# lrmantovani10/Stable-Diffusion.mojo

Hardware: AMD Instinct MI355X
Metric: UNet denoising steps/sec @ 512x512 latent, batch=8 (higher is better)
Workload: dtype f16; 1 GPU; Tiny-SD UNet 512x512 (latent 4x64x64), batch 8/GPU, 50-step DDPM schedule, 77-token context, no CFG, random-init weights (BASELINE configs[1]); global_batch=8, parallelism=dp1 (independent prompts, weights broadcast once)

## Files before the change

### include/tsd.h

```cpp
#ifndef TSD_H
#define TSD_H

#include <stddef.h>
#include <stdint.h>

#ifdef __cplusplus
extern "C" {
#endif

#define TSD_VERSION 100

typedef enum tsd_status {
  TSD_OK = 0,
  TSD_E_ARG = -1,
  TSD_E_SHAPE = -2,
  TSD_E_ALLOC = -3,
  TSD_E_HIP = -4,
  TSD_E_RCCL = -5,
  TSD_E_STATE = -6,
  TSD_E_NONFINITE = -7
} tsd_status;

typedef struct tsd_ctx tsd_ctx;
typedef struct tsd_model tsd_model;
// ... 166 lines not shown
};
#define TSD_GD_VERSION_1 1
enum tsd_gemm_operand { TSD_GO_A0 = 0, TSD_GO_A1, TSD_GO_A2, TSD_GO_W, TSD_GO_WT1, TSD_GO_R, TSD_GO_BIAS, TSD_GO_ROWVEC, TSD_GO_C,
                        TSD_GO_VT, TSD_GO_GN, TSD_GO_COUNT };
int tsd_debug_gemm_record(tsd_ctx* ctx, int on);
int tsd_debug_gemm_recorded(tsd_ctx* ctx, int i, int64_t* desc, int n);
int tsd_debug_gemm_run(tsd_ctx* ctx, const int64_t* desc, int n, int cfg, const void* const* host_in, void* const* host_out,
                       int64_t* ext, int64_t* info);
enum tsd_norm_desc_field {
  TSD_ND_VERSION = 0, TSD_ND_MODE, TSD_ND_B, TSD_ND_HW, TSD_ND_C, TSD_ND_C0, TSD_ND_LD0, TSD_ND_LD1, TSD_ND_LDY, TSD_ND_GROUPS,
  TSD_ND_EPS, TSD_ND_GAMMA, TSD_ND_SILU, TSD_ND_HAS_W, TSD_ND_HAS_B, TSD_ND_TORCH_RSTD,
  TSD_ND_STATS, TSD_ND_NSLAB, TSD_ND_G0, TSD_ND_G1, TSD_ND_COMB, TSD_ND_ROWS,
  TSD_ND_COUNT
};
#define TSD_ND_VERSION_1 1
enum tsd_norm_mode { TSD_NM_GROUPNORM = 0, TSD_NM_GN_STATS, TSD_NM_GN_FINALIZE, TSD_NM_LAYERNORM };
enum tsd_norm_operand { TSD_NO_X0 = 0, TSD_NO_X1, TSD_NO_PART0, TSD_NO_PART1, TSD_NO_W, TSD_NO_BIAS, TSD_NO_Y, TSD_NO_STATS, TSD_NO_COUNT };
enum tsd_norm_info { TSD_NI_CHANGED = 0, TSD_NI_NSLAB, TSD_NI_OWN_PASS, TSD_NI_PREREDUCE, TSD_NI_FINALIZE, TSD_NI_COMPOSITE,
                     TSD_NI_SLAB_PIXELS, TSD_NI_APPLY_PIXELS, TSD_NI_PL, TSD_NI_COUNT };
int tsd_debug_norm_run(tsd_ctx* ctx, const int64_t* desc, int n, const void* const* host_in, void* const* host_out, int64_t* ext,
                       int64_t* info);
int tsd_debug_gn_path_counts(tsd_ctx* ctx, int64_t* counts, int n, int reset);
int tsd_debug_model_fold(tsd_model* m, int block, void* wf, float* bf);
int tsd_debug_attn_bench(tsd_ctx* ctx, int B, int H, int d, int Sq, int Sk, int iters, float* ms);
int tsd_debug_attn_exact_passes(tsd_ctx* ctx, int reset);
int tsd_debug_set_attn_qb(tsd_ctx* ctx, int mode);
int tsd_debug_set_attn_diag(tsd_ctx* ctx, int on);
int tsd_debug_set_res_fuse_skip(tsd_ctx* ctx, int on);
int tsd_debug_set_qkv_fuse(tsd_ctx* ctx, int on);
int tsd_debug_set_session_hoist(tsd_ctx* ctx, int on);
int tsd_debug_session_hoist_info(tsd_session* s, int64_t* info);
int tsd_debug_mfma_sustained(tsd_ctx* ctx, float ms_target, float* tflops, float* clock_ghz);

double tsd_flop_count(int kind, int L, int T);

#ifdef __cplusplus
}
#endif
#endif
```

### stable-diffusion.mojo_amd/csrc/common.h

```cpp
#pragma once
#include <hip/hip_runtime.h>
#include <stdint.h>
#include <stdio.h>
#include <string>
#include <vector>

#include "../../include/tsd.h"
#include "counter_rng.h"

typedef _Float16 half_t;

void tsd_set_error(const char* fmt, ...);
#define TSD_FAIL(code, ...)      \
  do {                           \
    tsd_set_error(__VA_ARGS__);  \
    return (code);               \
  } while (0)
#define HIP_TRY(expr)                                                                              \
  do {                                                                                             \
    hipError_t e__ = (expr);                                                                       \
    if (e__ != hipSuccess) TSD_FAIL(TSD_E_HIP, "%s failed: %s (%s:%d)", #expr, hipGetErrorString(e__), __FILE__, __LINE__); \
  } while (0)
#define TSD_TRY(expr)            \
  do {                           \
// ... 4 lines not shown
struct Arena {
  char* base = nullptr;
  size_t cap = 0, top = 0, peak = 0;
  bool planning = false;
  size_t mark() const { return top; }
  void release(size_t m) { top = m; }
  void* alloc(size_t bytes) {
    size_t a = (top + 255) & ~size_t(255);
    size_t n = a + bytes;
    if (n > peak) peak = n;
    if (!planning && n > cap) return nullptr;
    top = n;
    return planning ? (void*)(uintptr_t)(0x1000 + a) : (void*)(base + a);
  }
};

struct TsdOptions {
  int qkv_fuse = 1;
  int res_fuse_skip = 1;
  int gn_composite = 1;
  int conv_in_im2col = 1;
  int chain = 1;
  int fold_out = 1;
  int session_hoist = 1;
  int conv_w_tm_mib = 2, lin_w_tm = 1, lin_w_tm_kib = 1024;
  int attn_qb = 2;
  int attn_qb_force = 0;
  int attn_wg8 = 1;
  int attn8_var = 0;
  int attn_diag = 1;
  int attn_xcd = 0;
  int xcdn = 0, conv_halo = 0, splitk = 1, splitk_mink = 4096, splitk_tiles = 256, splitk_small = 8, splitk_wide = 1, splitk_ring4 = 0,
      splitk_big = 0, sk_cfg = 5, thin_cfg = 0, tune = 15, sk256 = 0, skip128 = 1;
  int force_cfg = -1;
  int sk_big_graph = 0;
  char cfg_override[512] = "";
  int gn_apply_mult = 2;
  int gn_finalize_min = 2048;
  int debug_occ = 0;
  int debug_poison_what = 7;
  int debug_poison = -1;
  int bench_wrot = 1, bench_epi = 0, bench_altcfg = -1, gemm_ts = 0;
  unsigned gen = 0;
};
void options_from_env(TsdOptions& o);

// ... 287 lines not shown
```

### stable-diffusion.mojo_amd/csrc/graph.cpp

```cpp
#include <math.h>

#include "graph.h"

#define CHECK_ALLOC(p) \
  if (!(p)) TSD_FAIL(TSD_E_ALLOC, "workspace arena exhausted (%s:%d)", __FILE__, __LINE__)

static int zero_async(tsd_ctx* ctx, void* p, size_t bytes) {
  if (!ctx->launch()) return TSD_OK;
  HIP_TRY(hipMemsetAsync(p, 0, bytes, ctx->stream));
  return TSD_OK;
}

Act act_alloc_gn(tsd_ctx* ctx, int B, int H, int W, int C, int groups) {
  Act a = act_alloc(ctx, B, H, W, C);
  if (a.p && groups > 0 && C % groups == 0) {
    a.gn_buf = arena_alloc<float>(ctx, (int64_t)B * ceil_div(H * W, 32) * groups * 2);
    a.gn_groups = a.gn_buf ? groups : 0;
  }
  return a;
}

static void gn_emit(const tsd_ctx* ctx, GemmArgs& g, Act* dst, int rows_per_sample) {
  if (!dst || !dst->gn_buf || dst->gn_groups <= 0 || g.N != dst->C || (g.epi & (EPI_OUT_F32 | EPI_GEGLU))) return;
  const int ns = gemm_gnstats_slabs(ctx, g.M, g.N, g.K, g.batch, g.conv, rows_per_sample, dst->gn_groups);
// ... 67 lines not shown
}

static NormSrc norm_src(const CatSrc& x, int C) {
  NormSrc s;
  s.x0 = x.p0; s.ld0 = x.ld0; s.C0 = x.C0;
  if (x.p1 && C > x.C0) { s.x1 = x.p1; s.ld1 = x.ld1; }
  return s;
}

extern "C" int tsd_debug_set_res_fuse_skip(tsd_ctx* ctx, int on) {
  return ctx_set_option(ctx, &TsdOptions::res_fuse_skip, on, 0, 1);
}

int g_resblock(tsd_ctx* ctx, const CatSrc& x, int B, int Hin, int Win, int ups, const ResW& w, const float* tvec,
               int tld, Act& out) {
  const int cin = w.cin, cout = w.cout;
  if (cin % 64 || cout % 64) TSD_FAIL(TSD_E_SHAPE, "residual block: channels (%d,%d) must be multiples of 64", cin, cout);
  if (cin > x.C0 + (x.p1 ? x.C1 : 0)) TSD_FAIL(TSD_E_SHAPE, "residual block: input has fewer than %d channels", cin);
  if (x.p1 && cin > x.C0 && (x.C0 % 64)) TSD_FAIL(TSD_E_SHAPE, "residual block: concat split %d not a multiple of 64", x.C0);
  if (!w.has_skip && (ups || (x.p1 && cin > x.C0))) TSD_FAIL(TSD_E_SHAPE, "residual block: identity skip needs a plain input");
  const int H = ups ? 2 * Hin : Hin, W = ups ? 2 * Win : Win;
  const size_t mark = ctx->arena.mark();
  Act h = act_alloc(ctx, B, Hin, Win, cin); CHECK_ALLOC(h.p);
  const bool x_stats = !(x.p1 && cin > x.C0) && x.gn_part0 && x.gn_groups0 == w.groups && x.C0 == cin;
  GnComposite gc;
  if (ctx->opt.gn_composite && x.p1 && cin == x.C0 + x.C1 && x.gn_part0 && x.gn_part1 && x.gn_groups0 > 0 && x.gn_groups1 > 0 &&
      x.gn_nslab0 == x.gn_nslab1 && x.gn_nslab0 > 0 && x.C0 % x.gn_groups0 == 0 && x.C1 % x.gn_groups1 == 0 && cin % w.groups == 0) {
    const int cf = x.C0 / x.gn_groups0, cpg = cin / w.groups;
    if (cf == x.C1 / x.gn_groups1 && cpg % cf == 0) {
      gc.part0 = x.gn_part0; gc.G0 = x.gn_groups0; gc.part1 = x.gn_part1; gc.G1 = x.gn_groups1; gc.nslab = x.gn_nslab0; gc.comb = cpg / cf;
    }
  }
  TSD_TRY(launch_groupnorm(ctx, norm_src(x, cin), B, Hin * Win, cin, w.groups, w.eps, 1.f, 1, h.p, h.ld,
                           x_stats ? x.gn_part0 : nullptr, x.gn_nslab0, w.gn1.w ? &w.gn1 : nullptr, gc.part0 ? &gc : nullptr));
  Act t1 = act_alloc_gn(ctx, B, H, W, cout, w.groups); CHECK_ALLOC(t1.p);
  TSD_TRY(g_conv3x3(ctx, h, w.conv1, 1, 1, 1, ups, tvec ? tvec + w.time_off : nullptr, tld, nullptr, 0, false, t1.p, t1.ld, &t1));
  Act h3 = act_alloc(ctx, B, H, W, cout); CHECK_ALLOC(h3.p);
  TSD_TRY(launch_groupnorm(ctx, norm_src(cat1(t1), cout), B, H * W, cout, w.groups, w.eps, 1.f, 1, h3.p, h3.ld, t1.gn_part,
                           t1.gn_nslab, w.gn2.w ? &w.gn2 : nullptr));
  Act r;
  if (w.has_skip && !ups && ctx->opt.res_fuse_skip > 0 && w.skip.k == 1 && w.skip.Ipad % 64 == 0 && w.skip.Ipad == cin &&
      !(x.p1 && cin > x.C0 && (x.C0 % 64))) {
    TSD_TRY(g_conv3x3(ctx, h3, w.conv2, 1, 1, 1, 0, nullptr, 0, nullptr, 0, false, out.p, out.ld, &out, &x, &w.skip));
    ctx->arena.release(mark);
    return TSD_OK;
  }
  if (w.has_skip) {
    r = act_alloc(ctx, B, Hin, Win, cout); CHECK_ALLOC(r.p);
    TSD_TRY(g_linear(ctx, x, (int64_t)B * Hin * Win, w.skip.w, w.skip.Ipad, cout, w.skip.Ipad, w.skip.b, nullptr, 0, 0,
                     r.p, r.ld));
  } else {
    r.p = const_cast<half_t*>(x.p0); r.ld = x.ld0; r.B = B; r.H = Hin; r.W = Win; r.C = cout;
  }
  TSD_TRY(g_conv3x3(ctx, h3, w.conv2, 1, 1, 1, 0, nullptr, 0, &r, ups, false, out.p, out.ld, &out));
  ctx->arena.release(mark);
  return TSD_OK;
// ... 313 lines not shown
  }
  auto attn = [&](int i) -> int {
    TSD_TRY(alloc_out(i, a[i - 1].H, a[i - 1].C));
    const AttnW& w = u.attn[i - 1];
    CtxKV kv;
    kv.K = kc_all + w.kv_off; kv.ldk = CK; kv.sK = (int64_t)Tp * CK;
    kv.Vt = vtc_all + (int64_t)w.kv_off * Tp; kv.ldvt = Tp; kv.sVt = (int64_t)CK * Tp;
    return g_unet_attn(ctx, a[i - 1], w, ctx16, T, Tp, a[i], &kv);
  };
  TSD_TRY(alloc_out(1, L, 320));
  if (in_im2col) TSD_TRY(g_linear(ctx, cat1(x0), (int64_t)B * L * L, u.conv_in_im2col, 64, u.conv1.Opad, 64, u.conv1.b, nullptr, 0, 0, a[1].p,
                                  a[1].ld, &a[1], L * L));
  else TSD_TRY(g_conv3x3(ctx, x0, u.conv1, 1, 1, 1, 0, nullptr, 0, nullptr, 0, false, a[1].p, a[1].ld, &a[1]));
  TSD_TRY(res(2, cat1(a[1]), L, 0));
  TSD_TRY(attn(3));
  TSD_TRY(alloc_out(4, L1, 320));
  TSD_TRY(g_conv3x3(ctx, a[3], u.conv4, 2, 1, 1, 0, nullptr, 0, nullptr, 0, false, a[4].p, a[4].ld, &a[4]));
  TSD_TRY(res(5, cat1(a[4]), L1, 0));
  TSD_TRY(attn(6));
  TSD_TRY(alloc_out(7, L2, 640));
  TSD_TRY(g_conv3x3(ctx, a[6], u.conv7, 2, 1, 1, 0, nullptr, 0, nullptr, 0, false, a[7].p, a[7].ld, &a[7]));
  TSD_TRY(res(8, cat1(a[7]), L2, 0));
  TSD_TRY(attn(9));
  TSD_TRY(res(10, cat2(a[9], a[9]), L2, 0));
  TSD_TRY(attn(11));
  TSD_TRY(res(12, cat2(a[11], a[7]), L2, 0));
  TSD_TRY(attn(13));
  TSD_TRY(res(15, cat1(a[13]), L2, 1));
  a[14] = a[15];
  TSD_TRY(attn(16));
  TSD_TRY(res(17, cat2(a[16], a[4]), L1, 0));
  TSD_TRY(attn(18));
  TSD_TRY(res(20, cat1(a[18]), L1, 1));
  a[19] = a[20];
  TSD_TRY(attn(21));
  TSD_TRY(res(22, cat2(a[21], a[1]), L, 0));
  TSD_TRY(attn(23));
  Act hf = act_alloc(ctx, B, L, L, 320); CHECK_ALLOC(hf.p);
  TSD_TRY(launch_groupnorm(ctx, norm_src(cat1(a[23]), 320), B, L * L, 320, 320, 1e-5f, 1.f, 1, hf.p, hf.ld,
                           a[23].gn_groups == 320 ? a[23].gn_part : nullptr, a[23].gn_nslab));
  if (eps_nhwc && u.final_conv.Opad == 4)
    return g_conv3x3(ctx, hf, u.final_conv, 1, 1, 1, 0, nullptr, 0, nullptr, 0, true, eps_out_chw, 4);
  float* eps_tmp = arena_alloc<float>(ctx, (int64_t)B * L * L * 4); CHECK_ALLOC(eps_tmp);
  TSD_TRY(g_conv3x3(ctx, hf, u.final_conv, 1, 1, 1, 0, nullptr, 0, nullptr, 0, true, eps_tmp, 4));
  TSD_TRY(launch_nhwc_f32_to_chw_f32(ctx, eps_tmp, B, 4, L, L, 4, eps_out_chw));
  return TSD_OK;
// ... 249 lines not shown
```

### stable-diffusion.mojo_amd/csrc/model.cpp

```cpp
#include <math.h>
#include <string.h>

#include "model.h"

bool attn_tail_weights_ok(const AttnW& w) {
  const int C = w.C;
  const bool plain = !w.ln[1].w && !w.ln[1].b && !w.ln[2].w && !w.ln[2].b && !w.gelu_erf;
  return plain && C == 320 && w.n_head == 8 && w.n_embed == 40 && w.sa_out.b && w.ca_out.b && w.geglu1.b && w.geglu2.b &&
         w.conv_out.b && !w.ca_q.b && w.sa_out.Kpad == C && w.ca_q.Kpad == C && w.ca_out.Kpad == C && w.geglu1.Kpad == C &&
         w.geglu2.Kpad == 4 * C && w.conv_out.Ipad == C && w.conv_out.k == 1;
}

bool attn_head_weights_ok(const AttnW& w) {
  const int C = w.C;
  return C == 320 && w.n_head == 8 && w.n_embed == 40 && !w.gn.w && !w.gn.b && !w.ln[0].w && !w.ln[0].b && w.conv_in.b &&
         w.conv_in.k == 1 && w.conv_in.Ipad == C && w.conv_in.Opad == C && !w.sa_in.b && w.sa_in.Kpad == C && w.sa_in.N == 3 * C;
}

static void model_invalidate_derived(tsd_model* m) {
  m->ready = false;
  m->gen++;
  for (auto& a : m->unet.attn) { a.tail_stream = nullptr; a.head_stream = nullptr; a.fold_w = nullptr; a.fold_w_tm = nullptr; a.fold_b = nullptr; }
  m->unet.conv_in_im2col = nullptr;
  m->vae.conv_in_im2col = nullptr;
  for (auto& r : m->unet.res) { r.conv1.w_tm = nullptr; r.conv2.w_tm = nullptr; }
  m->unet.conv4.w_tm = nullptr; m->unet.conv7.w_tm = nullptr; m->unet.kproj_all.w_tm = nullptr;
  for (auto& cv : m->unet.conv) cv.w_tm = nullptr;
  for (auto& a : m->unet.attn) {
    for (LinW* l : {&a.sa_in, &a.sa_out, &a.ca_q, &a.ca_out, &a.geglu1, &a.geglu2}) l->w_tm = nullptr;
    a.conv_in.w_tm = nullptr; a.conv_out.w_tm = nullptr;
  }
}

static size_t packed_bytes(const ParamSpec& p) {
  if (!p.used) return 0;
  switch (p.kind) {
    case P_CONV_W: return (size_t)p.Opad * p.shape[2] * p.shape[3] * p.Kpad * sizeof(half_t);
    case P_CONV_B: return (size_t)p.Opad * sizeof(float);
    case P_LIN_W: return (size_t)p.shape[0] * p.Kpad * sizeof(half_t);
    default: return (size_t)p.shape[0] * sizeof(float);
  }
}

extern "C" int tsd_model_create(tsd_ctx* ctx, int kind, tsd_model** out) {
// ... 126 lines not shown
      if (m->derived) HIP_TRY(hipFree(m->derived));
      m->derived = nullptr; m->derived_bytes = 0;
      hipError_t e = hipMalloc((void**)&m->derived, need);
      if (e != hipSuccess) TSD_FAIL(TSD_E_ALLOC, "derived weights: hipMalloc(%zu) failed: %s", need, hipGetErrorString(e));
      m->derived_bytes = need;
      if (ctx->opt.debug_poison >= 0 && (ctx->opt.debug_poison_what & 2)) HIP_TRY(hipMemsetAsync(m->derived, ctx->opt.debug_poison & 255, need, ctx->stream));
    }
    const bool wp = ctx->arena.planning;
    ctx->arena.planning = false;
    const int r = launch_pack_im2col_w(ctx, c0.w, c0.Opad, c0.Ipad, c0.I, (half_t*)m->derived);
    ctx->arena.planning = wp;
    if (r == TSD_OK) m->vae.conv_in_im2col = (const half_t*)m->derived;
    return r;
  }
  if (!is_diffusion_kind(m->kind)) return TSD_OK;
  std::vector<AttnW*> el;
  for (auto& a : m->unet.attn) if (a.C && (attn_tail_weights_ok(a) || attn_head_weights_ok(a))) el.push_back(&a);
  const ConvW& cin = is_full_unet_kind(m->kind) ? (m->unet.conv.empty() ? m->unet.conv1 : m->unet.conv[0]) : m->unet.conv1;
  const bool cin_ok = cin.w && cin.k == 3 && cin.I > 0 && 9 * cin.I <= 64 && cin.Ipad == 64;
  const size_t cin_b = cin_ok ? ((size_t)cin.Opad * 64 * sizeof(half_t) + 255) & ~size_t(255) : 0;
  const int tm_mib = ctx->opt.conv_w_tm_mib;
  const int tml_kib = ctx->opt.lin_w_tm_kib;
  const size_t tml_bytes = (size_t)(tml_kib > 0 ? tml_kib : 1024) << 10;
  std::vector<ConvW*> tm;
  size_t tm_b = 0;
  if (tm_mib > 0)
    for (auto& r : m->unet.res)
      for (ConvW* c : {&r.conv1, &r.conv2})
        if (c->w && c->k == 3 && (size_t)c->Opad * 9 * c->Ipad * 2 >= (size_t)tm_mib << 20) { tm.push_back(c); tm_b += (((size_t)c->Opad * 9 * c->Ipad * 2) + 255) & ~size_t(255); }
  if (tm_mib > 0) {
    for (ConvW* c : {&m->unet.conv4, &m->unet.conv7})
      if (c->w && c->k == 3 && (size_t)c->Opad * 9 * c->Ipad * 2 >= (size_t)tm_mib << 20) { tm.push_back(c); tm_b += (((size_t)c->Opad * 9 * c->Ipad * 2) + 255) & ~size_t(255); }
    for (auto& cv : m->unet.conv)
      if (cv.w && cv.k == 3 && (size_t)cv.Opad * 9 * cv.Ipad * 2 >= (size_t)tm_mib << 20) { tm.push_back(&cv); tm_b += (((size_t)cv.Opad * 9 * cv.Ipad * 2) + 255) & ~size_t(255); }
  }
  if (tm_mib > 0 && ctx->opt.lin_w_tm != 0)
    for (auto& a : m->unet.attn)
      if (a.C && !(attn_tail_weights_ok(a) && attn_head_weights_ok(a)))
        for (ConvW* c : {&a.conv_in, &a.conv_out})
          if (c->w && c->k == 1 && c->Ipad % 64 == 0 && (size_t)c->Opad * c->Ipad * 2 >= tml_bytes) { tm.push_back(c); tm_b += (((size_t)c->Opad * c->Ipad * 2) + 255) & ~size_t(255); }
  const int tml_mib = ctx->opt.lin_w_tm;
  std::vector<LinW*> tml;
  if (tml_mib > 0)
    for (auto& a : m->unet.attn)
      if (a.C && !(attn_tail_weights_ok(a) && attn_head_weights_ok(a)))
        for (LinW* l : {&a.sa_in, &a.sa_out, &a.ca_q, &a.ca_out, &a.geglu1, &a.geglu2})
          if (l->w && l->Kpad % 64 == 0 && l->Kpad == l->K && (size_t)l->N * l->Kpad * 2 >= tml_bytes) { tml.push_back(l); tm_b += (((size_t)l->N * l->Kpad * 2) + 255) & ~size_t(255); }
  LinW* kv = nullptr;
  if (tml_mib > 0 && m->unet.kproj_all.w && m->unet.vproj_all.w == m->unet.kproj_all.w + (int64_t)m->unet.kproj_all.N * m->unet.kproj_all.Kpad &&
      m->unet.kproj_all.Kpad % 64 == 0 && m->unet.vproj_all.N == m->unet.kproj_all.N) {
    kv = &m->unet.kproj_all;
    tm_b += (((size_t)2 * kv->N * kv->Kpad * 2) + 255) & ~size_t(255);
  }
  std::vector<AttnW*> fold;
  size_t fold_b = 0;
  if (ctx->opt.fold_out)
    for (auto& a : m->unet.attn)
      if (a.C && !attn_tail_weights_ok(a) && a.geglu2.w && a.conv_out.w && a.conv_out.k == 1 && a.conv_out.Ipad == a.C && a.conv_out.Opad == a.C &&
          a.geglu2.N == a.C && a.geglu2.Kpad == 4 * a.C && a.geglu2.K == 4 * a.C && a.C % 64 == 0) {
        fold.push_back(&a);
        fold_b += 2 * ((((size_t)a.C * 5 * a.C * 2) + 255) & ~size_t(255)) + ((((size_t)a.C * 4) + 255) & ~size_t(255));
      }
  if (el.empty() && !cin_ok && tm.empty() && tml.empty() && !kv && fold.empty()) return TSD_OK;
  const size_t tail_b = (attn_tail_stream_bytes() + 255) & ~size_t(255), head_b = (attn_head_stream_bytes() + 255) & ~size_t(255);
  const size_t each = tail_b + head_b, need = each * el.size() + cin_b + tm_b + fold_b;
  HIP_TRY(hipSetDevice(ctx->device));
  if (m->derived_bytes < need) {
    if (m->derived) HIP_TRY(hipFree(m->derived));
    m->derived = nullptr; m->derived_bytes = 0;
    hipError_t e = hipMalloc((void**)&m->derived, need);
    if (e != hipSuccess) TSD_FAIL(TSD_E_ALLOC, "derived weights: hipMalloc(%zu) failed: %s", need, hipGetErrorString(e));
    m->derived_bytes = need;
    if (ctx->opt.debug_poison >= 0 && (ctx->opt.debug_poison_what & 2)) HIP_TRY(hipMemsetAsync(m->derived, ctx->opt.debug_poison & 255, need, ctx->stream));
  }
  const bool was_planning = ctx->arena.planning;
  ctx->arena.planning = false;
  int r = TSD_OK;
  for (size_t i = 0; i < el.size() && r == TSD_OK; i++) {
    AttnW& a = *el[i];
    half_t* dst = (half_t*)(m->derived + i * each);
    if (attn_tail_weights_ok(a)) {
      r = launch_attn_tail_pack(ctx, a.sa_out.w, a.sa_out.Kpad, a.ca_q.w, a.ca_q.Kpad, a.ca_out.w, a.ca_out.Kpad, a.geglu1.w,
                                a.geglu1.Kpad, a.geglu2.w, a.geglu2.Kpad, a.conv_out.w, a.conv_out.Ipad, dst);
      if (r == TSD_OK) a.tail_stream = dst;
    }
    if (r == TSD_OK && attn_head_weights_ok(a)) {
      half_t* hd = (half_t*)(m->derived + i * each + tail_b);
      r = launch_attn_head_pack(ctx, a.conv_in.w, a.conv_in.Ipad, a.sa_in.w, a.sa_in.Kpad, hd);
// ... 18 lines not shown
      half_t* dst = (half_t*)(m->derived + off);
      r = launch_pack_tile_major(ctx, kv->w, 2 * kv->N, kv->Kpad, dst);
      if (r == TSD_OK) kv->w_tm = dst;
      off += (((size_t)2 * kv->N * kv->Kpad * 2) + 255) & ~size_t(255);
    }
    for (size_t i = 0; i < tml.size() && r == TSD_OK; i++) {
      LinW* l = tml[i];
      half_t* dst = (half_t*)(m->derived + off);
      r = launch_pack_tile_major(ctx, l->w, l->N, l->Kpad, dst);
      if (r == TSD_OK) l->w_tm = dst;
      off += (((size_t)l->N * l->Kpad * 2) + 255) & ~size_t(255);
    }
    for (size_t i = 0; i < fold.size() && r == TSD_OK; i++) {
      AttnW* a = fold[i];
      const int C = a->C;
      const size_t wb = (((size_t)C * 5 * C * 2) + 255) & ~size_t(255);
      half_t* wf = (half_t*)(m->derived + off);
      half_t* wf_tm = (half_t*)(m->derived + off + wb);
      float* bf = (float*)(m->derived + off + 2 * wb);
      r = launch_fold_linear_conv1x1(ctx, a->conv_out.w, a->conv_out.Ipad, a->conv_out.b, a->geglu2.w, a->geglu2.Kpad, a->geglu2.b, C, 4 * C, wf, 5 * C, bf);
      if (r == TSD_OK) r = launch_pack_tile_major(ctx, wf, C, 5 * C, wf_tm);
      if (r == TSD_OK) { a->fold_w = wf; a->fold_w_tm = wf_tm; a->fold_b = bf; }
      off += 2 * wb + ((((size_t)C * 4) + 255) & ~size_t(255));
    }
  }
  if (r == TSD_OK && !fold.empty()) {
    hipError_t e = hipStreamSynchronize(ctx->stream);
    for (size_t i = 0; i < fold.size() && r == TSD_OK && e == hipSuccess; i++) {
      const AttnW* a = fold[i];
      const int C = a->C;
      std::vector<uint16_t> hw((size_t)C * 5 * C);
      std::vector<float> hb(C);
      e = hipMemcpy(hw.data(), a->fold_w, hw.size() * 2, hipMemcpyDeviceToHost);
      if (e == hipSuccess) e = hipMemcpy(hb.data(), a->fold_b, hb.size() * 4, hipMemcpyDeviceToHost);
      if (e != hipSuccess) break;
      int64_t bad = 0;
      for (uint16_t v : hw) bad += (v & 0x7C00) == 0x7C00;
      for (float v : hb) bad += !(fabsf(v) <= 3.4028235e38f);
      if (bad) {
        fold[i]->fold_w = nullptr; fold[i]->fold_w_tm = nullptr; fold[i]->fold_b = nullptr;
        tsd_set_error("attention block with C = %d: %lld folded weights / biases are not finite (W_out . W_2 leaves fp16)", C, (long long)bad);
        r = TSD_E_NONFINITE;
      }
    }
    if (e != hipSuccess && r == TSD_OK) {
      tsd_set_error("fold check: %s", hipGetErrorString(e));
// ... 14 lines not shown
  return TSD_OK;
}

extern "C" int tsd_model_prepare(tsd_model* m) {
  if (!m) TSD_FAIL(TSD_E_ARG, "NULL model");
  HIP_TRY(hipSetDevice(m->ctx->device));
  TSD_TRY(model_check_ready(m));
  HIP_TRY(hipStreamSynchronize(m->ctx->stream));
  return TSD_OK;
}

extern "C" int tsd_debug_model_fold(tsd_model* m, int block, void* wf, float* bf) {
  if (!m) TSD_FAIL(TSD_E_ARG, "NULL model");
  if (!is_diffusion_kind(m->kind) || block < 0 || block >= (int)m->unet.attn.size())
    TSD_FAIL(TSD_E_ARG, "model_fold: no attention block %d in this model", block);
  HIP_TRY(hipSetDevice(m->ctx->device));
  TSD_TRY(model_check_ready(m));
  const AttnW& a = m->unet.attn[block];
  if (!a.fold_w) return 0;
  HIP_TRY(hipStreamSynchronize(m->ctx->stream));
  if (wf) HIP_TRY(hipMemcpy(wf, a.fold_w, (size_t)a.C * 5 * a.C * 2, hipMemcpyDeviceToHost));
  if (bf) HIP_TRY(hipMemcpy(bf, a.fold_b, (size_t)a.C * 4, hipMemcpyDeviceToHost));
  return a.C;
}

ConvW model_conv(const tsd_model* m, const std::string& prefix) {
  ConvW w;
  auto it = m->index.find(prefix + ".kernel");
  if (it == m->index.end()) return w;
  const ParamSpec& pw = m->params[it->second];
  const ParamSpec& pb = m->params[it->second + 1];
  if (!pw.used) return w;
  w.w = (const half_t*)(m->blob + pw.off);
  w.b = (const float*)(m->blob + pb.off);
  w.O = (int)pw.shape[0]; w.I = (int)pw.shape[1]; w.k = (int)pw.shape[2]; w.Ipad = pw.Kpad; w.Opad = pw.Opad;
  return w;
}

LinW model_lin(const tsd_model* m, const std::string& prefix, bool use_bias) {
  LinW w;
  auto it = m->index.find(prefix + ".weight");
  if (it == m->index.end()) return w;
  const ParamSpec& pw = m->params[it->second];
  const ParamSpec& pb = m->params[it->second + 1];
  w.w = (const half_t*)(m->blob + pw.off);
  w.b = (use_bias && pb.used) ? (const float*)(m->blob + pb.off) : nullptr;
// ... 141 lines not shown
```

### stable-diffusion.mojo_amd/csrc/model.h

```cpp
#pragma once
#include <map>
#include <string>
#include <vector>

#include "common.h"

enum ParamKind { P_CONV_W = 0, P_CONV_B = 1, P_LIN_W = 2, P_LIN_B = 3 };

struct ParamSpec {
  std::string name;
  int64_t shape[4] = {0, 0, 0, 0};
  int ndim = 0;
  int kind = 0;
  bool used = true;
  float bound = 0.f;
  float offset = 0.f;
  int Opad = 0, Kpad = 0;
  int interleave = 0;
  int region = 0;
  size_t off = 0, bytes = 0;
  int64_t numel() const {
    int64_t n = 1;
    for (int i = 0; i < ndim; i++) n *= shape[i];
    return n;
// ... 3 lines not shown
enum LayerKind { L_CONV, L_CONV_S2, L_RES, L_ATTN, L_UP, L_GN, L_SILU, L_UPCONV };
struct LayerDef { int kind; int a, b, c, d; };
extern const LayerDef UNET_LAYERS[23];
extern const LayerDef DECODER_LAYERS[26];
extern const LayerDef ENCODER_LAYERS[19];
enum { U_POP = 1, U_PUSH = 2 };
struct UNetStep { LayerDef l; int flags; };
constexpr int SD15_N = 45;
extern const UNetStep SD15_STEPS[SD15_N];
static inline bool is_full_unet_kind(int kind) { return kind == TSD_MODEL_DIFFUSION_SD15 || kind == TSD_MODEL_DIFFUSION_SD15_TORCH; }
static inline bool is_diffusion_kind(int kind) { return kind == TSD_MODEL_DIFFUSION || is_full_unet_kind(kind); }
static inline bool is_clip_kind(int kind) { return kind == TSD_MODEL_CLIP || kind == TSD_MODEL_CLIP_TORCH; }
static inline bool is_decoder_kind(int kind) { return kind == TSD_MODEL_DECODER || kind == TSD_MODEL_DECODER_TORCH; }
static inline bool is_encoder_kind(int kind) { return kind == TSD_MODEL_ENCODER || kind == TSD_MODEL_ENCODER_TORCH; }
static inline bool is_vae_torch_kind(int kind) { return kind == TSD_MODEL_DECODER_TORCH || kind == TSD_MODEL_ENCODER_TORCH; }
constexpr int TSD_MODEL_KIND_MAX = TSD_MODEL_ENCODER_TORCH;

std::vector<ParamSpec> build_param_specs(int model_kind);

struct ResW {
  ConvW conv1, conv2, skip;
  LinW time;
  int cin = 0, cout = 0, groups = 32;
  bool has_skip = false;
  int time_off = 0;
  NormAffine gn1, gn2;
  float eps = 1e-5f;
};
struct AttnW {
  int n_head = 0, n_embed = 0, C = 0, d_ctx = 768;
  ConvW conv_in, conv_out;
  LinW sa_in, sa_out, ca_q, ca_k, ca_v, ca_out, geglu1, geglu2;
  int kv_off = 0;
  NormAffine gn, ln[3];
  bool gelu_erf = false;
  const half_t* tail_stream = nullptr;
  const half_t* head_stream = nullptr;
  const half_t* fold_w = nullptr; const half_t* fold_w_tm = nullptr; const float* fold_b = nullptr;
};
bool attn_tail_weights_ok(const AttnW& w);
bool attn_head_weights_ok(const AttnW& w);
struct VaeAttnW {
  int C = 0;
  LinW in_proj, out_proj;
  NormAffine gn;
  float eps = 1e-5f;
};

struct UNetW {
  LinW t1, t2;
  LinW tproj;
  LinW kproj_all, vproj_all;
  ConvW conv1, conv4, conv7, final_conv;
  const half_t* conv_in_im2col = nullptr;
  std::vector<ResW> res;
  std::vector<AttnW> attn;
  std::vector<ConvW> conv;
  NormAffine final_gn;
  int final_groups = 320;
};
struct VaeW {
  std::vector<ConvW> conv;
  const half_t* conv_in_im2col = nullptr;
  std::vector<ResW> res;
  std::vector<VaeAttnW> attn;
  std::vector<NormAffine> gn;
  float gn_eps = 1e-5f;
};

struct ClipLayerW { LinW in_proj, out_proj, l4, l5; NormAffine ln1, ln2; };
struct ClipW {
  const half_t* tok = nullptr;
  const float* pos = nullptr;
  ClipLayerW layer[12];
  NormAffine final_ln;
};

struct PlanKey { int B, L, T; bool operator<(const PlanKey& o) const { return B != o.B ? B < o.B : (L != o.L ? L < o.L : T < o.T); } };

struct tsd_model {
// ... 22 lines not shown
```

### stable-diffusion.mojo_amd/csrc/runtime.cpp

```cpp
#include <stdarg.h>
#include <stdlib.h>
#include <string.h>

#include "common.h"

static thread_local char g_err[512] = "";

void tsd_set_error(const char* fmt, ...) {
  va_list ap;
  va_start(ap, fmt);
  vsnprintf(g_err, sizeof(g_err), fmt, ap);
  va_end(ap);
}

static int env_int(const char* name, int dflt) { const char* e = getenv(name); return e && *e ? atoi(e) : dflt; }
void options_from_env(TsdOptions& o) {
  o.qkv_fuse = env_int("TSD_QKV_FUSE", o.qkv_fuse);
  o.res_fuse_skip = env_int("TSD_RES_FUSE_SKIP", o.res_fuse_skip);
  o.gn_composite = env_int("TSD_GN_COMPOSITE", o.gn_composite);
  o.conv_in_im2col = env_int("TSD_CONV_IN_IM2COL", o.conv_in_im2col);
  o.chain = env_int("TSD_CHAIN", o.chain) ? 1 : 0;
  o.fold_out = env_int("TSD_FOLD_OUT", o.fold_out) ? 1 : 0;
  o.session_hoist = env_int("TSD_SESSION_HOIST", o.session_hoist) ? 1 : 0;
  o.conv_w_tm_mib = env_int("TSD_CONV_W_TM", o.conv_w_tm_mib);
  o.lin_w_tm = env_int("TSD_LIN_W_TM", o.lin_w_tm);
  o.lin_w_tm_kib = env_int("TSD_LIN_W_TM_KIB", o.lin_w_tm_kib);
  { const int q = env_int("TSD_ATTN_QB", o.attn_qb); if (q == 1 || q == 2) o.attn_qb = q; }
  o.attn_xcd = env_int("TSD_ATTN_XCD", o.attn_xcd);
  o.attn_wg8 = env_int("TSD_ATTN_WG8", o.attn_wg8) ? 1 : 0;
  o.attn8_var = env_int("TSD_ATTN8_VAR", o.attn8_var);
  o.xcdn = env_int("TSD_GEMM_XCDN", o.xcdn);
  o.conv_halo = env_int("TSD_CONV_HALO", o.conv_halo);
  o.splitk = env_int("TSD_GEMM_SPLITK", o.splitk);
  o.splitk_mink = env_int("TSD_GEMM_SPLITK_MINK", o.splitk_mink);
  o.splitk_tiles = env_int("TSD_GEMM_SPLITK_TILES", o.splitk_tiles);
  o.splitk_small = env_int("TSD_GEMM_SPLITK_SMALL", o.splitk_small);
  o.splitk_wide = env_int("TSD_GEMM_SPLITK_WIDE", o.splitk_wide);
  o.splitk_ring4 = env_int("TSD_GEMM_SPLITK_RING4", o.splitk_ring4);
  o.splitk_big = env_int("TSD_GEMM_SPLITK_BIG", o.splitk_big);
  o.sk_cfg = env_int("TSD_GEMM_SK_CFG", o.sk_cfg);
  o.sk256 = env_int("TSD_GEMM_SK256", o.sk256);
  o.thin_cfg = env_int("TSD_GEMM_THIN_CFG", o.thin_cfg);
  o.skip128 = env_int("TSD_GEMM_SKIP128", o.skip128);
  o.tune = env_int("TSD_GEMM_TUNE", o.tune);
  if (const char* ov = getenv("TSD_GEMM_CFG_OVERRIDE")) { strncpy(o.cfg_override, ov, sizeof(o.cfg_override) - 1); o.cfg_override[sizeof(o.cfg_override) - 1] = 0; }
// ... 185 lines not shown
```

### stable-diffusion.mojo_amd/tsd/_lib.py

```python
import ctypes as C
import os

import numpy as np

_HERE = os.path.dirname(os.path.abspath(__file__))
LIB_PATH = os.environ.get("TSD_LIB") or os.path.join(os.path.dirname(_HERE), "lib", "libtsd.so")

TSD_OK, TSD_E_ARG, TSD_E_SHAPE, TSD_E_ALLOC, TSD_E_HIP, TSD_E_RCCL, TSD_E_STATE, TSD_E_NONFINITE = 0, -1, -2, -3, -4, -5, -6, -7
os.environ.setdefault("HIP_FORCE_DEV_KERNARG", "1")

MODEL_DIFFUSION, MODEL_DECODER, MODEL_ENCODER, MODEL_CLIP, MODEL_DIFFUSION_SD15, MODEL_DIFFUSION_SD15_TORCH = 1, 2, 3, 4, 5, 6
MODEL_CLIP_TORCH, MODEL_DECODER_TORCH, MODEL_ENCODER_TORCH = 7, 8, 9
SAMPLER_KINDS = {"ddpm": 0, "ddim": 1, "dpmpp_2m": 2}
TIMESTEP_SPACINGS = {"leading": 0, "trailing": 1}
MASK_MODES = {"area": 0, "any": 1}


def sampler_kind(kind):
    return SAMPLER_KINDS.get(kind.lower(), -1) if isinstance(kind, str) else int(kind)


def timestep_spacing(spacing):
    return TIMESTEP_SPACINGS.get(spacing.lower(), -1) if isinstance(spacing, str) else int(spacing)

# ... 92 lines not shown
        "tsd_session_download_latents": ([vp, fp], i), "tsd_session_download_images": ([vp, i, fp], i),
        "tsd_dist_unique_id": ([vp], i), "tsd_dist_init": ([vp, i, i, vp], i),
        "tsd_dist_broadcast_weights": ([vp, i], i), "tsd_dist_finalize": ([vp], i),
        "tsd_dist_comm_count": ([vp, C.POINTER(i)], i),
        "tsd_flop_count": ([i, i, i], C.c_double),
        "tsd_debug_splitk_errors": ([vp], i),
        "tsd_debug_xcd_round_robin": ([], i),
        "tsd_debug_nonfinite_count": ([vp, i], i),
        "tsd_debug_set_fused_attention": ([vp, i], i),
        "tsd_debug_gemm_bench": ([vp, i, i, i, i, i, i, i, i, i, i, fp], i),
        "tsd_debug_attn_bench": ([vp, i, i, i, i, i, i, fp], i),
        "tsd_debug_attn_exact_passes": ([vp, i], i),
        "tsd_debug_set_attn_qb": ([vp, i], i),
        "tsd_debug_set_attn_diag": ([vp, i], i),
        "tsd_debug_set_res_fuse_skip": ([vp, i], i),
        "tsd_debug_set_qkv_fuse": ([vp, i], i),
        "tsd_debug_set_session_hoist": ([vp, i], i),
        "tsd_debug_session_hoist_info": ([vp, C.POINTER(i64)], i),
        "tsd_debug_mfma_sustained": ([vp, C.c_float, fp, fp], i),
        "tsd_debug_gemm_check": ([vp, i, i, i, i, i, i, i, i, i, i, fp, fp], i),
        "tsd_debug_gemm_record": ([vp, i], i),
        "tsd_debug_gemm_recorded": ([vp, i, C.POINTER(i64), i], i),
        "tsd_debug_model_fold": ([vp, i, vp, fp], i),
        "tsd_debug_gemm_run": ([vp, C.POINTER(i64), i, i, C.POINTER(vp), C.POINTER(vp), C.POINTER(i64), C.POINTER(i64)], i),
        "tsd_debug_norm_run": ([vp, C.POINTER(i64), i, C.POINTER(vp), C.POINTER(vp), C.POINTER(i64), C.POINTER(i64)], i),
        "tsd_debug_gn_path_counts": ([vp, C.POINTER(i64), i, i], i),
    }
    for name, (args, res) in sig.items():
        fn = getattr(l, name)
        fn.argtypes = args
        fn.restype = res


EXPORTS = None


def declared_symbols():
    import re
    hdr = os.path.join(os.path.dirname(os.path.dirname(_HERE)), "include", "tsd.h")
    txt = open(hdr).read()
    txt = re.sub(r"/\*.*?\*/", "", txt, flags=re.S)
    return sorted(set(re.findall(r"\b(tsd_[a-z0-9_]+)\s*\(", txt)))


def last_error():
    return lib().tsd_last_error().decode()
# ... 84 lines not shown
```

Before: 213.5 steps/s.

## Fold duplicated-concat residual block weights to halve input channels

In the Tiny-SD UNet, layer 10's residual block takes cat(a9, a9), the same activation concatenated with itself. The change sums the two input-channel halves of the conv1 and skip weights on the host at model prep time, and sets groups_in to half the groups. The block then runs on a9 alone with half the input channels, which removes half the GEMM K work and the concat read for that block. GroupNorm on the duplicated input is equivalent with half the groups, and it can reuse upstream stats through a new composite path. The costs are one-time host prep, extra derived weight memory, and fp16 rounding of the summed weights.

Result: faster. 217.0 steps/s, median of 6 (+1.6%).

```diff
diff --git a/include/tsd.h b/include/tsd.h
--- a/include/tsd.h
+++ b/include/tsd.h
@@ -212,6 +212,8 @@
                        int64_t* info);
 int tsd_debug_gn_path_counts(tsd_ctx* ctx, int64_t* counts, int n, int reset);
 int tsd_debug_model_fold(tsd_model* m, int block, void* wf, float* bf);
+int tsd_debug_model_dup_fold(tsd_model* m, void* conv1_w, void* skip_w);
+int64_t tsd_debug_dup_fold_host(const void* w, int rows, int taps, int ldw, int half, void* out, int ldo);
 int tsd_debug_attn_bench(tsd_ctx* ctx, int B, int H, int d, int Sq, int Sk, int iters, float* ms);
 int tsd_debug_attn_exact_passes(tsd_ctx* ctx, int reset);
 int tsd_debug_set_attn_qb(tsd_ctx* ctx, int mode);
diff --git a/stable-diffusion.mojo_amd/csrc/common.h b/stable-diffusion.mojo_amd/csrc/common.h
--- a/stable-diffusion.mojo_amd/csrc/common.h
+++ b/stable-diffusion.mojo_amd/csrc/common.h
@@ -50,6 +50,7 @@
   int conv_in_im2col = 1;
   int chain = 1;
   int fold_out = 1;
+  int fold_dup = 1;
   int session_hoist = 1;
   int conv_w_tm_mib = 2, lin_w_tm = 1, lin_w_tm_kib = 1024;
   int attn_qb = 2;
diff --git a/stable-diffusion.mojo_amd/csrc/graph.cpp b/stable-diffusion.mojo_amd/csrc/graph.cpp
--- a/stable-diffusion.mojo_amd/csrc/graph.cpp
+++ b/stable-diffusion.mojo_amd/csrc/graph.cpp
@@ -113,16 +113,20 @@
   const int H = ups ? 2 * Hin : Hin, W = ups ? 2 * Win : Win;
   const size_t mark = ctx->arena.mark();
   Act h = act_alloc(ctx, B, Hin, Win, cin); CHECK_ALLOC(h.p);
-  const bool x_stats = !(x.p1 && cin > x.C0) && x.gn_part0 && x.gn_groups0 == w.groups && x.C0 == cin;
+  const int g_in = w.groups_in > 0 ? w.groups_in : w.groups;
+  const bool x_stats = !(x.p1 && cin > x.C0) && x.gn_part0 && x.gn_groups0 == g_in && x.C0 == cin;
   GnComposite gc;
   if (ctx->opt.gn_composite && x.p1 && cin == x.C0 + x.C1 && x.gn_part0 && x.gn_part1 && x.gn_groups0 > 0 && x.gn_groups1 > 0 &&
-      x.gn_nslab0 == x.gn_nslab1 && x.gn_nslab0 > 0 && x.C0 % x.gn_groups0 == 0 && x.C1 % x.gn_groups1 == 0 && cin % w.groups == 0) {
-    const int cf = x.C0 / x.gn_groups0, cpg = cin / w.groups;
+      x.gn_nslab0 == x.gn_nslab1 && x.gn_nslab0 > 0 && x.C0 % x.gn_groups0 == 0 && x.C1 % x.gn_groups1 == 0 && cin % g_in == 0) {
+    const int cf = x.C0 / x.gn_groups0, cpg = cin / g_in;
     if (cf == x.C1 / x.gn_groups1 && cpg % cf == 0) {
       gc.part0 = x.gn_part0; gc.G0 = x.gn_groups0; gc.part1 = x.gn_part1; gc.G1 = x.gn_groups1; gc.nslab = x.gn_nslab0; gc.comb = cpg / cf;
     }
-  }
-  TSD_TRY(launch_groupnorm(ctx, norm_src(x, cin), B, Hin * Win, cin, w.groups, w.eps, 1.f, 1, h.p, h.ld,
+  } else if (ctx->opt.gn_composite && !x_stats && !(x.p1 && cin > x.C0) && x.C0 == cin && x.gn_part0 && x.gn_nslab0 > 0 && x.gn_groups0 > g_in &&
+             x.gn_groups0 % g_in == 0 && cin % x.gn_groups0 == 0) {
+    gc.part0 = x.gn_part0; gc.G0 = x.gn_groups0; gc.nslab = x.gn_nslab0; gc.comb = x.gn_groups0 / g_in;
+  }
+  TSD_TRY(launch_groupnorm(ctx, norm_src(x, cin), B, Hin * Win, cin, g_in, w.eps, 1.f, 1, h.p, h.ld,
                            x_stats ? x.gn_part0 : nullptr, x.gn_nslab0, w.gn1.w ? &w.gn1 : nullptr, gc.part0 ? &gc : nullptr));
   Act t1 = act_alloc_gn(ctx, B, H, W, cout, w.groups); CHECK_ALLOC(t1.p);
   TSD_TRY(g_conv3x3(ctx, h, w.conv1, 1, 1, 1, ups, tvec ? tvec + w.time_off : nullptr, tld, nullptr, 0, false, t1.p, t1.ld, &t1));
@@ -482,6 +486,10 @@
   TSD_TRY(g_conv3x3(ctx, a[6], u.conv7, 2, 1, 1, 0, nullptr, 0, nullptr, 0, false, a[7].p, a[7].ld, &a[7]));
   TSD_TRY(res(8, cat1(a[7]), L2, 0));
   TSD_TRY(attn(9));
+  if (u.res_dup_on && ctx->opt.fold_dup && a[9].C == u.res_dup.cin) {
+    TSD_TRY(alloc_out(10, L2, u.res_dup.cout));
+    TSD_TRY(g_resblock(ctx, cat1(a[9]), B, L2, L2, 0, u.res_dup, tvec, tld, a[10]));
+  } else
   TSD_TRY(res(10, cat2(a[9], a[9]), L2, 0));
   TSD_TRY(attn(11));
   TSD_TRY(res(12, cat2(a[11], a[7]), L2, 0));
diff --git a/stable-diffusion.mojo_amd/csrc/model.cpp b/stable-diffusion.mojo_amd/csrc/model.cpp
--- a/stable-diffusion.mojo_amd/csrc/model.cpp
+++ b/stable-diffusion.mojo_amd/csrc/model.cpp
@@ -17,9 +17,69 @@
          w.conv_in.k == 1 && w.conv_in.Ipad == C && w.conv_in.Opad == C && !w.sa_in.b && w.sa_in.Kpad == C && w.sa_in.N == 3 * C;
 }
 
+static double f16_bits_to_f64(uint16_t h) {
+  const uint64_t sign = (uint64_t)(h & 0x8000) << 48;
+  const int e = (h >> 10) & 31;
+  const uint64_t m = h & 0x3FF;
+  uint64_t u;
+  if (e == 31) u = sign | (0x7FFull << 52) | (m << 42);
+  else if (e == 0) {
+    const double v = ldexp((double)m, -24);
+    return sign ? -v : v;
+  } else u = sign | ((uint64_t)(e - 15 + 1023) << 52) | (m << 42);
+  double d;
+  memcpy(&d, &u, 8);
+  return d;
+}
+
+static uint16_t f64_to_f16_bits_rne(double v) {
+  uint64_t u;
+  memcpy(&u, &v, 8);
+  const uint16_t sign = (uint16_t)((u >> 48) & 0x8000);
+  const int e = (int)((u >> 52) & 0x7FF);
+  uint64_t m = u & ((1ull << 52) - 1);
+  if (e == 0x7FF) {
+    uint16_t r = (uint16_t)(0x7C00 + (m >> 42));
+    if (m && r == 0x7C00) r++;
+    return sign | r;
+  }
+  if (e == 0) return sign;
+  const int E = e - 1023;
+  m |= 1ull << 52;
+  const int shift = 42 + (E < -14 ? -14 - E : 0);
+  if (shift > 63) return sign;
+  uint64_t q = m >> shift;
+  const uint64_t rem = m & ((1ull << shift) - 1), half = 1ull << (shift - 1);
+  if (rem > half || (rem == half && (q & 1))) q++;
+  uint64_t bits = E >= -14 ? ((uint64_t)(E + 14) << 10) + q : q;
+  if (bits >= 0x7C00) bits = 0x7C00;
+  return sign | (uint16_t)bits;
+}
+
+static int64_t dup_fold_host(const uint16_t* w, int64_t rows, int taps, int ldw, int half, uint16_t* out, int ldo) {
+  int64_t bad = 0;
+  for (int64_t rt = 0; rt < rows * taps; rt++) {
+    const uint16_t* s = w + rt * ldw;
+    uint16_t* d = out + rt * ldo;
+    for (int c = 0; c < half; c++) {
+      const uint16_t a = s[c], b = s[half + c];
+      d[c] = f64_to_f16_bits_rne(f16_bits_to_f64(a) + f16_bits_to_f64(b));
+      bad += (d[c] & 0x7C00) == 0x7C00;
+    }
+    for (int c = half; c < ldo; c++) d[c] = 0;
+  }
+  return bad;
+}
+
+extern "C" int64_t tsd_debug_dup_fold_host(const void* w, int rows, int taps, int ldw, int half, void* out, int ldo) {
+  if (!w || !out || rows <= 0 || taps <= 0 || half <= 0 || ldw < 2 * half || ldo < half) TSD_FAIL(TSD_E_ARG, "dup_fold_host: bad argument");
+  return dup_fold_host((const uint16_t*)w, rows, taps, ldw, half, (uint16_t*)out, ldo);
+}
+
 static void model_invalidate_derived(tsd_model* m) {
   m->ready = false;
   m->gen++;
+  m->unet.res_dup_on = false; m->unet.res_dup = ResW();
   for (auto& a : m->unet.attn) { a.tail_stream = nullptr; a.head_stream = nullptr; a.fold_w = nullptr; a.fold_w_tm = nullptr; a.fold_b = nullptr; }
   m->unet.conv_in_im2col = nullptr;
   m->vae.conv_in_im2col = nullptr;
@@ -192,12 +252,27 @@
   const int tm_mib = ctx->opt.conv_w_tm_mib;
   const int tml_kib = ctx->opt.lin_w_tm_kib;
   const size_t tml_bytes = (size_t)(tml_kib > 0 ? tml_kib : 1024) << 10;
+  bool dup = false;
+  if (ctx->opt.fold_dup && !is_full_unet_kind(m->kind) && m->unet.res.size() > 9 && m->unet.attn.size() > 8) {
+    const ResW& r = m->unet.res[9];
+    const int half = r.cin / 2;
+    dup = r.cin > 0 && r.cin % 2 == 0 && half % 64 == 0 && m->unet.attn[8].C == half && r.groups % 2 == 0 && half % (r.groups / 2) == 0 &&
+          r.conv1.w && r.conv1.k == 3 && r.conv1.Ipad == r.cin && r.has_skip && r.skip.w && r.skip.k == 1 && r.skip.Ipad == r.cin &&
+          r.skip.Opad == r.conv1.Opad && !r.gn1.w && !r.gn1.b;
+  }
+  size_t dup_w1_b = 0, dup_sk_b = 0, dup_tm_b = 0;
+  if (dup) {
+    const ResW& r = m->unet.res[9];
+    dup_w1_b = (((size_t)r.conv1.Opad * 9 * (r.cin / 2) * 2) + 255) & ~size_t(255);
+    dup_sk_b = (((size_t)r.skip.Opad * (r.cin / 2) * 2) + 255) & ~size_t(255);
+    if (tm_mib > 0 && (size_t)r.conv1.Opad * 9 * (r.cin / 2) * 2 >= (size_t)tm_mib << 20) dup_tm_b = dup_w1_b;
+  }
   std::vector<ConvW*> tm;
   size_t tm_b = 0;
   if (tm_mib > 0)
     for (auto& r : m->unet.res)
       for (ConvW* c : {&r.conv1, &r.conv2})
-        if (c->w && c->k == 3 && (size_t)c->Opad * 9 * c->Ipad * 2 >= (size_t)tm_mib << 20) { tm.push_back(c); tm_b += (((size_t)c->Opad * 9 * c->Ipad * 2) + 255) & ~size_t(255); }
+        if (!(dup && c == &m->unet.res[9].conv1) && c->w && c->k == 3 && (size_t)c->Opad * 9 * c->Ipad * 2 >= (size_t)tm_mib << 20) { tm.push_back(c); tm_b += (((size_t)c->Opad * 9 * c->Ipad * 2) + 255) & ~size_t(255); }
   if (tm_mib > 0) {
     for (ConvW* c : {&m->unet.conv4, &m->unet.conv7})
       if (c->w && c->k == 3 && (size_t)c->Opad * 9 * c->Ipad * 2 >= (size_t)tm_mib << 20) { tm.push_back(c); tm_b += (((size_t)c->Opad * 9 * c->Ipad * 2) + 255) & ~size_t(255); }
@@ -231,9 +306,9 @@
         fold.push_back(&a);
         fold_b += 2 * ((((size_t)a.C * 5 * a.C * 2) + 255) & ~size_t(255)) + ((((size_t)a.C * 4) + 255) & ~size_t(255));
       }
-  if (el.empty() && !cin_ok && tm.empty() && tml.empty() && !kv && fold.empty()) return TSD_OK;
+  if (el.empty() && !cin_ok && tm.empty() && tml.empty() && !kv && fold.empty() && !dup) return TSD_OK;
   const size_t tail_b = (attn_tail_stream_bytes() + 255) & ~size_t(255), head_b = (attn_head_stream_bytes() + 255) & ~size_t(255);
-  const size_t each = tail_b + head_b, need = each * el.size() + cin_b + tm_b + fold_b;
+  const size_t each = tail_b + head_b, need = each * el.size() + cin_b + tm_b + fold_b + dup_w1_b + dup_sk_b + dup_tm_b;
   HIP_TRY(hipSetDevice(ctx->device));
   if (m->derived_bytes < need) {
     if (m->derived) HIP_TRY(hipFree(m->derived));
@@ -298,6 +373,45 @@
       if (r == TSD_OK) r = launch_pack_tile_major(ctx, wf, C, 5 * C, wf_tm);
       if (r == TSD_OK) { a->fold_w = wf; a->fold_w_tm = wf_tm; a->fold_b = bf; }
       off += 2 * wb + ((((size_t)C * 4) + 255) & ~size_t(255));
+    }
+    if (dup && r == TSD_OK) {
+      const ResW& r10 = m->unet.res[9];
+      const int half = r10.cin / 2;
+      const size_t n1 = (size_t)r10.conv1.Opad * 9 * r10.cin, ns = (size_t)r10.skip.Opad * r10.cin;
+      std::vector<uint16_t> src(std::max(n1, ns)), dst(std::max(n1, ns) / 2);
+      half_t* w1 = (half_t*)(m->derived + off);
+      half_t* wsk = (half_t*)(m->derived + off + dup_w1_b);
+      half_t* w1_tm = dup_tm_b ? (half_t*)(m->derived + off + dup_w1_b + dup_sk_b) : nullptr;
+      off += dup_w1_b + dup_sk_b + dup_tm_b;
+      int64_t bad = 0;
+      hipError_t e = hipStreamSynchronize(ctx->stream);
+      for (int k = 0; k < 2 && e == hipSuccess; k++) {
+        const ConvW& c = k ? r10.skip : r10.conv1;
+        const size_t n = k ? ns : n1;
+        e = hipMemcpy(src.data(), c.w, n * 2, hipMemcpyDeviceToHost);
+        if (e != hipSuccess) break;
+        bad += dup_fold_host(src.data(), c.Opad, c.k * c.k, c.Ipad, half, dst.data(), half);
+        e = hipMemcpyAsync(k ? wsk : w1, dst.data(), n, hipMemcpyHostToDevice, ctx->stream);
+        if (e == hipSuccess) e = hipStreamSynchronize(ctx->stream);
+      }
+      if (e != hipSuccess) {
+        tsd_set_error("duplicate-concat fold: %s", hipGetErrorString(e));
+        r = TSD_E_HIP;
+      } else if (bad) {
+        tsd_set_error("unet.layer10: %lld folded conv1 / skip weights are not finite (the sum of the two input-channel halves leaves fp16)",
+                      (long long)bad);
+        r = TSD_E_NONFINITE;
+      } else {
+        ResW d = r10;
+        d.cin = half; d.groups_in = r10.groups / 2;
+        d.conv1.w = w1; d.conv1.I = half; d.conv1.Ipad = half; d.conv1.w_tm = nullptr;
+        d.skip.w = wsk; d.skip.I = half; d.skip.Ipad = half; d.skip.w_tm = nullptr;
+        if (w1_tm) {
+          r = launch_pack_tile_major(ctx, w1, d.conv1.Opad, 9 * half, w1_tm);
+          if (r == TSD_OK) d.conv1.w_tm = w1_tm;
+        }
+        if (r == TSD_OK) { m->unet.res_dup = d; m->unet.res_dup_on = true; }
+      }
     }
   }
   if (r == TSD_OK && !fold.empty()) {
@@ -358,6 +472,19 @@
   if (wf) HIP_TRY(hipMemcpy(wf, a.fold_w, (size_t)a.C * 5 * a.C * 2, hipMemcpyDeviceToHost));
   if (bf) HIP_TRY(hipMemcpy(bf, a.fold_b, (size_t)a.C * 4, hipMemcpyDeviceToHost));
   return a.C;
+}
+
+extern "C" int tsd_debug_model_dup_fold(tsd_model* m, void* conv1_w, void* skip_w) {
+  if (!m) TSD_FAIL(TSD_E_ARG, "NULL model");
+  if (!is_diffusion_kind(m->kind)) TSD_FAIL(TSD_E_ARG, "model_dup_fold: not a diffusion model");
+  HIP_TRY(hipSetDevice(m->ctx->device));
+  TSD_TRY(model_check_ready(m));
+  if (!m->unet.res_dup_on) return 0;
+  const ResW& d = m->unet.res_dup;
+  HIP_TRY(hipStreamSynchronize(m->ctx->stream));
+  if (conv1_w) HIP_TRY(hipMemcpy(conv1_w, d.conv1.w, (size_t)d.conv1.Opad * 9 * d.conv1.Ipad * 2, hipMemcpyDeviceToHost));
+  if (skip_w) HIP_TRY(hipMemcpy(skip_w, d.skip.w, (size_t)d.skip.Opad * d.skip.Ipad * 2, hipMemcpyDeviceToHost));
+  return d.cin;
 }
 
 ConvW model_conv(const tsd_model* m, const std::string& prefix) {
diff --git a/stable-diffusion.mojo_amd/csrc/model.h b/stable-diffusion.mojo_amd/csrc/model.h
--- a/stable-diffusion.mojo_amd/csrc/model.h
+++ b/stable-diffusion.mojo_amd/csrc/model.h
@@ -49,6 +49,7 @@
   ConvW conv1, conv2, skip;
   LinW time;
   int cin = 0, cout = 0, groups = 32;
+  int groups_in = 0;
   bool has_skip = false;
   int time_off = 0;
   NormAffine gn1, gn2;
@@ -83,6 +84,8 @@
   std::vector<ResW> res;
   std::vector<AttnW> attn;
   std::vector<ConvW> conv;
+  ResW res_dup;
+  bool res_dup_on = false;
   NormAffine final_gn;
   int final_groups = 320;
 };
diff --git a/stable-diffusion.mojo_amd/csrc/runtime.cpp b/stable-diffusion.mojo_amd/csrc/runtime.cpp
--- a/stable-diffusion.mojo_amd/csrc/runtime.cpp
+++ b/stable-diffusion.mojo_amd/csrc/runtime.cpp
@@ -21,6 +21,7 @@
   o.conv_in_im2col = env_int("TSD_CONV_IN_IM2COL", o.conv_in_im2col);
   o.chain = env_int("TSD_CHAIN", o.chain) ? 1 : 0;
   o.fold_out = env_int("TSD_FOLD_OUT", o.fold_out) ? 1 : 0;
+  o.fold_dup = env_int("TSD_FOLD_DUP", o.fold_dup) ? 1 : 0;
   o.session_hoist = env_int("TSD_SESSION_HOIST", o.session_hoist) ? 1 : 0;
   o.conv_w_tm_mib = env_int("TSD_CONV_W_TM", o.conv_w_tm_mib);
   o.lin_w_tm = env_int("TSD_LIN_W_TM", o.lin_w_tm);
diff --git a/stable-diffusion.mojo_amd/tsd/_lib.py b/stable-diffusion.mojo_amd/tsd/_lib.py
--- a/stable-diffusion.mojo_amd/tsd/_lib.py
+++ b/stable-diffusion.mojo_amd/tsd/_lib.py
@@ -138,6 +138,8 @@
         "tsd_debug_gemm_record": ([vp, i], i),
         "tsd_debug_gemm_recorded": ([vp, i, C.POINTER(i64), i], i),
         "tsd_debug_model_fold": ([vp, i, vp, fp], i),
+        "tsd_debug_model_dup_fold": ([vp, vp, vp], i),
+        "tsd_debug_dup_fold_host": ([vp, i, i, i, i, vp, i], i64),
         "tsd_debug_gemm_run": ([vp, C.POINTER(i64), i, i, C.POINTER(vp), C.POINTER(vp), C.POINTER(i64), C.POINTER(i64)], i),
         "tsd_debug_norm_run": ([vp, C.POINTER(i64), i, C.POINTER(vp), C.POINTER(vp), C.POINTER(i64), C.POINTER(i64)], i),
         "tsd_debug_gn_path_counts": ([vp, C.POINTER(i64), i, i], i),
```
